# codelion/adaptive-classifier

Measured on NVIDIA B200. Metric: queries/sec predict() bert-base 128-tok, 1M x 768 prototypes, higher is better.
Workload: dtype f16

## Files before the change

### adaptive_classifier_b200/csrc/api.cu

```cuda
#include "common.cuh"
#include <cstdarg>
#include <cudaTypedefs.h>
#include <atomic>
#include <mutex>
#include <vector>

namespace ac {

static thread_local char g_err[512] = "";

void set_error(const char *fmt, ...) {
    va_list ap;
    va_start(ap, fmt);
    vsnprintf(g_err, sizeof(g_err), fmt, ap);
    va_end(ap);
}

int check_cuda(cudaError_t e, const char *what) {
    if (e == cudaSuccess) return AC_OK;
    set_error("CUDA error %d (%s) at %s", static_cast<int>(e), cudaGetErrorString(e), what);
    return AC_E_CUDA;
}

static std::atomic<long long> g_launches{0};
// ... 50 lines not shown
        if (cudaGetDevice(&dev) != cudaSuccess) return 148;
        if (cudaDeviceGetAttribute(&n, cudaDevAttrMultiProcessorCount, dev) != cudaSuccess || n <= 0) n = 148;
    }
    return n;
}

int make_tmap_2d(CUtensorMap *out, const void *gptr, int elem_bytes, uint64_t rows, uint64_t cols,
                 uint64_t row_stride_bytes, uint32_t box_rows, uint32_t box_cols) {
    static PFN_cuTensorMapEncodeTiled_v12000 encode = nullptr;
    static std::once_flag once;
    std::call_once(once, [] {
        void *fn = nullptr;
        cudaDriverEntryPointQueryResult qres;
        if (cudaGetDriverEntryPoint("cuTensorMapEncodeTiled", &fn, cudaEnableDefault, &qres) == cudaSuccess &&
            qres == cudaDriverEntryPointSuccess)
            encode = reinterpret_cast<PFN_cuTensorMapEncodeTiled_v12000>(fn);
    });
    if (!encode) {
        set_error("cuTensorMapEncodeTiled entry point not available (no CUDA driver?)");
        return AC_E_CUDA;
    }
    AC_REQUIRE((reinterpret_cast<uintptr_t>(gptr) & 15) == 0 && row_stride_bytes % 16 == 0,
               "make_tmap_2d: base pointer and row stride must be 16-byte aligned");
    AC_REQUIRE(box_cols * static_cast<uint32_t>(elem_bytes) == 128 && box_rows <= 256,
               "make_tmap_2d: box must be 128 bytes wide and <= 256 rows");
    const CUtensorMapDataType dt = (elem_bytes == 4) ? CU_TENSOR_MAP_DATA_TYPE_FLOAT32 : CU_TENSOR_MAP_DATA_TYPE_FLOAT16;
    cuuint64_t gdim[2] = {cols, rows};
    cuuint64_t gstride[1] = {row_stride_bytes};
    cuuint32_t box[2] = {box_cols, box_rows};
    cuuint32_t estr[2] = {1, 1};
    CUresult r = encode(out, dt, 2, const_cast<void *>(gptr), gdim, gstride, box, estr, CU_TENSOR_MAP_INTERLEAVE_NONE,
                        CU_TENSOR_MAP_SWIZZLE_128B, CU_TENSOR_MAP_L2_PROMOTION_L2_256B,
                        CU_TENSOR_MAP_FLOAT_OOB_FILL_NONE);
    if (r != CUDA_SUCCESS) {
        set_error("cuTensorMapEncodeTiled failed with CUresult %d (rows=%llu cols=%llu)", static_cast<int>(r),
                  static_cast<unsigned long long>(rows), static_cast<unsigned long long>(cols));
        return AC_E_CUDA;
    }
    return AC_OK;
}

int launch_knn_dist_exact(const float *Q, const float *P, int nq, int64_t N, int D, float *Dout, cudaStream_t stream);
int launch_knn_rerank(const float *Q, const float *P, int B, int64_t N, int D, int kc, const int32_t *cand, float *out_d,
                      int64_t *out_i, int64_t row_offset, cudaStream_t stream);
size_t topk_select_workspace(int B, int64_t L, int k);
int topk_select(const float *d, const int64_t *idx, int B, int64_t L, int64_t in_stride, int64_t id_offset, int k,
                float *out_d, int64_t *out_i, void *ws, size_t ws_bytes, cudaStream_t stream, const float *row_gate = nullptr);
size_t knn_tc_workspace(int B, int64_t N, int D, int k);
int knn_tc_search(const float *Q, const float *P, const float *p_sqnorm, const void *p_half, int B, int64_t N, int D, int k,
                  float *out_d, int64_t *out_i, int64_t row_offset, void *ws, size_t ws_bytes, int32_t *stats, cudaStream_t stream);

static int exact_query_block(int B, int64_t N) {
    const int64_t budget = 256ll << 20;
    int64_t qb = budget / (4 * (N > 0 ? N : 1));
    if (qb < 1) qb = 1;
// ... 120 lines not shown
```

### adaptive_classifier_b200/csrc/common.cuh

```cuda
#pragma once

#include <cuda_runtime.h>
#include <cuda.h>
#include <stdint.h>
#include <stdio.h>
#include <string.h>
#include <string>

#include "../../include/adaptive_b200.h"

namespace ac {

void set_error(const char *fmt, ...);
int check_cuda(cudaError_t e, const char *what);

#define AC_CUDA(call)                                                \
    do {                                                             \
        int _rc = ::ac::check_cuda((call), #call);                   \
        if (_rc != 0) return _rc;                                    \
    } while (0)

#define AC_REQUIRE(cond, ...)                                        \
    do {                                                             \
        if (!(cond)) {                                               \
// ... 21 lines not shown

__device__ __forceinline__ uint32_t smem_u32(const void *p) {
    return static_cast<uint32_t>(__cvta_generic_to_shared(p));
}

__device__ __forceinline__ float round_tf32(float x) {
    uint32_t u = __float_as_uint(x);
    u += 0x0FFFu + ((u >> 13) & 1u);
    u &= 0xFFFFE000u;
    return __uint_as_float(u);
}

__device__ __forceinline__ float warp_sum(float v) {
#pragma unroll
    for (int o = 16; o > 0; o >>= 1) v += __shfl_xor_sync(0xffffffffu, v, o);
    return v;
}
__device__ __forceinline__ float warp_max(float v) {
#pragma unroll
    for (int o = 16; o > 0; o >>= 1) v = fmaxf(v, __shfl_xor_sync(0xffffffffu, v, o));
    return v;
}

__device__ __forceinline__ void mbar_init(uint64_t *bar, uint32_t count) {
    asm volatile("mbarrier.init.shared::cta.b64 [%0], %1;" ::"r"(smem_u32(bar)), "r"(count));
}
__device__ __forceinline__ void fence_mbar_init() {
    asm volatile("fence.mbarrier_init.release.cluster;" ::: "memory");
}
__device__ __forceinline__ void mbar_arrive_expect_tx(uint64_t *bar, uint32_t bytes) {
    asm volatile("mbarrier.arrive.expect_tx.shared::cta.b64 _, [%0], %1;" ::"r"(smem_u32(bar)), "r"(bytes)
                 : "memory");
}
__device__ __forceinline__ void mbar_arrive(uint64_t *bar) {
    asm volatile("mbarrier.arrive.shared::cta.b64 _, [%0];" ::"r"(smem_u32(bar)) : "memory");
}
__device__ __forceinline__ bool mbar_try_wait(uint64_t *bar, uint32_t parity) {
    uint32_t ok;
    asm volatile(
        "{\n\t"
        ".reg .pred p;\n\t"
        "mbarrier.try_wait.parity.shared::cta.b64 p, [%1], %2;\n\t"
        "selp.u32 %0, 1, 0, p;\n\t"
        "}"
        : "=r"(ok)
        : "r"(smem_u32(bar)), "r"(parity)
        : "memory");
    return ok != 0;
}
__device__ __forceinline__ void mbar_wait(uint64_t *bar, uint32_t parity) {
    while (!mbar_try_wait(bar, parity)) {
    }
}

__device__ __forceinline__ void tma_prefetch_desc(const CUtensorMap *m) {
    asm volatile("prefetch.tensormap [%0];" ::"l"(reinterpret_cast<uint64_t>(m)) : "memory");
}
__device__ __forceinline__ void tma_load_2d(void *smem_dst, const CUtensorMap *m, uint64_t *bar, int c0, int c1) {
    asm volatile(
        "cp.async.bulk.tensor.2d.shared::cluster.global.tile.mbarrier::complete_tx::bytes [%0], [%1, {%3, %4}], [%2];"
        ::"r"(smem_u32(smem_dst)), "l"(reinterpret_cast<uint64_t>(m)), "r"(smem_u32(bar)), "r"(c0), "r"(c1)
        : "memory");
}
__device__ __forceinline__ void fence_proxy_async_smem() {
    asm volatile("fence.proxy.async.shared::cta;" ::: "memory");
}

__device__ __forceinline__ void tmem_alloc(uint32_t *smem_dst, uint32_t ncols) {
    asm volatile("tcgen05.alloc.cta_group::1.sync.aligned.shared::cta.b32 [%0], %1;" ::"r"(smem_u32(smem_dst)),
                 "r"(ncols)
                 : "memory");
}
__device__ __forceinline__ void tmem_relinquish() {
    asm volatile("tcgen05.relinquish_alloc_permit.cta_group::1.sync.aligned;" ::: "memory");
}
__device__ __forceinline__ void tmem_dealloc(uint32_t taddr, uint32_t ncols) {
    asm volatile("tcgen05.dealloc.cta_group::1.sync.aligned.b32 %0, %1;" ::"r"(taddr), "r"(ncols) : "memory");
}
__device__ __forceinline__ void tc_fence_before() { asm volatile("tcgen05.fence::before_thread_sync;" ::: "memory"); }
__device__ __forceinline__ void tc_fence_after() { asm volatile("tcgen05.fence::after_thread_sync;" ::: "memory"); }

__device__ __forceinline__ void tc_commit(uint64_t *bar) {
    asm volatile("tcgen05.commit.cta_group::1.mbarrier::arrive::one.shared::cluster.b64 [%0];" ::"r"(smem_u32(bar))
                 : "memory");
}

__device__ __forceinline__ uint64_t umma_desc_sw128(uint32_t smem_addr) {
    uint64_t d = 0;
    d |= static_cast<uint64_t>((smem_addr & 0x3FFFFu) >> 4);
// ... 134 lines not shown
```

### adaptive_classifier_b200/csrc/encoder.cu

```cuda
#include "gemm_tc2.cuh"
#include <cuda_fp16.h>
#include <math_constants.h>
#include <vector>

namespace ac {

__device__ __forceinline__ float ex2_approx(float x) {
    float y;
    asm("ex2.approx.ftz.f32 %0, %1;" : "=f"(y) : "f"(x));
    return y;
}
__device__ __forceinline__ float rcp_approx(float x) {
    float y;
    asm("rcp.approx.ftz.f32 %0, %1;" : "=f"(y) : "f"(x));
    return y;
}
__device__ __forceinline__ float gelu_erf(float y) {
    const float ay = fabsf(y);
    const float t = rcp_approx(fmaf(0.3275911f * 0.70710678118654752440f, ay, 1.f));
    float p = fmaf(0.5f * 1.061405429f, t, 0.5f * -1.453152027f);
    p = fmaf(p, t, 0.5f * 1.421413741f);
    p = fmaf(p, t, 0.5f * -0.284496736f);
    p = fmaf(p, t, 0.5f * 0.254829592f);
    const float e = ex2_approx((y * y) * (-0.5f * 1.4426950408889634f));
    const float h = (p * t) * e;
    return fmaxf(y, 0.f) - fabsf(y * h);
}

template <int MODE, bool OUT_HALF, bool VT, bool DEFER = false, int COLS = GEMM_BLOCK_N / 2>
struct EpiLinear {
    static_assert(!DEFER || (OUT_HALF && MODE != 2), "the deferred-LayerNorm consumer epilogues write fp16 operands");
    const float *__restrict__ bias;
    const float *__restrict__ residual;
    void *Y;
    int M, N, ldy;
    int round_out;
    __half *vT;
    int vt_col0, S, S_pad, H;
    const float *__restrict__ c1;
    const float2 *__restrict__ row_stats;

    static constexpr int kUnrollChunks = 4;
    static constexpr int kPrefetchDist = 1;
    struct State {
        float4 res[(MODE == 2) ? 2 : 1][(MODE == 2) ? 8 : 1];
        float mu, r;
    };
    __device__ __forceinline__ float pre(const State &st, float acc, float b, float c1v) const {
        return DEFER ? fmaf(st.r, fmaf(-st.mu, c1v, acc), b) : acc + b;
    }
    __device__ __forceinline__ void begin_cta(State &, int, int) const {}
    __device__ __forceinline__ void end_cta(State &, int, int) const {}

    __device__ __forceinline__ float act(float y) const {
        if (MODE == 1) y = gelu_erf(y);
        return y;
    }

    __device__ __forceinline__ void prefetch(State &st, const GemmTileInfo &ti, int row, int col0, int lane, int buf) const {
        if (DEFER) {
            if (((col0 - ti.n0) & (COLS - 1)) == 0) {
                const float2 ms = (row < M) ? __ldg(row_stats + row) : make_float2(0.f, 0.f);
                st.mu = ms.x;
                st.r = ms.y;
            }
        }
// ... 83 lines not shown
                const float4 b4 = (col + 4 <= N) ? __ldg(reinterpret_cast<const float4 *>(bias + col)) : make_float4(0, 0, 0, 0);
#pragma unroll
                for (int i = 0; i < 4; ++i) {
                    const int rr = r8 + 8 * i;
                    const int grow = row_base + rr;
                    if (grow < M && col + 4 <= N) {
                        const float4 a = *reinterpret_cast<const float4 *>(stage + rr * GEMM_EPI_STAGE_ROW_BYTES + 16 * c);
                        float4 o;
                        o.x = act(a.x + b4.x); o.y = act(a.y + b4.y); o.z = act(a.z + b4.z); o.w = act(a.w + b4.w);
                        if (MODE == 2) {
                            const float4 rs = st.res[buf][half * 4 + i];
                            o.x += rs.x; o.y += rs.y; o.z += rs.z; o.w += rs.w;
                        }
                        if (round_out) { o.x = round_tf32(o.x); o.y = round_tf32(o.y); o.z = round_tf32(o.z); o.w = round_tf32(o.w); }
                        *reinterpret_cast<float4 *>(Yf + static_cast<int64_t>(grow) * ldy + col) = o;
                    }
                }
                __syncwarp();
            }
        }
    }
};

struct EpiResidDefer {
    const float *__restrict__ bias;
    float *y;
    __half *yh;
    const float2 *__restrict__ stats_prev;
    const float *__restrict__ gamma;
    const float *__restrict__ beta;
    float2 *parts;
    int64_t part_stride;
    int M, N, ld;

    static constexpr int kUnrollChunks = 4;
#ifndef AC_RESID_PREFETCH
#define AC_RESID_PREFETCH 1
#endif
    static constexpr int kPrefetchDist = AC_RESID_PREFETCH;
    struct State {
        float4 res[kPrefetchDist + 1][8];
        float2 ms[4];
        float sum[4], sq[4];
    };
    __device__ __forceinline__ void begin_cta(State &, int, int) const {}
    __device__ __forceinline__ void end_cta(State &, int, int) const {}

    __device__ __forceinline__ void prefetch(State &st, const GemmTileInfo &ti, int, int col0, int lane, int buf) const {
        const int row_base = ti.m0 + ((threadIdx.x >> 5) & 3) * 32;
        const int r8 = lane >> 2, c = lane & 3;
        if (((col0 - ti.n0) & (GEMM_BLOCK_N / 2 - 1)) == 0) {
#pragma unroll
            for (int i = 0; i < 4; ++i) {
                const int grow = row_base + r8 + 8 * i;
                st.ms[i] = (grow < M) ? __ldg(stats_prev + grow) : make_float2(0.f, 0.f);
                st.sum[i] = 0.f;
                st.sq[i] = 0.f;
            }
        }
#pragma unroll
        for (int half = 0; half < 2; ++half) {
            const int col = col0 + 16 * half + 4 * c;
// ... 45 lines not shown
                    *reinterpret_cast<uint2 *>(yh + static_cast<int64_t>(grow) * ld + col) = pk;
                    st.sum[i] += (o.x + o.y) + (o.z + o.w);
                    st.sq[i] += (o.x * o.x + o.y * o.y) + (o.z * o.z + o.w * o.w);
                }
            }
            __syncwarp();
        }
        if (((col0 - ti.n0) & (GEMM_BLOCK_N / 2 - 1)) == GEMM_BLOCK_N / 2 - 32) {
            const int part = col0 / (GEMM_BLOCK_N / 2);
#pragma unroll
            for (int i = 0; i < 4; ++i) {
                float s = st.sum[i], q = st.sq[i];
                s += __shfl_xor_sync(0xffffffffu, s, 1);
                q += __shfl_xor_sync(0xffffffffu, q, 1);
                s += __shfl_xor_sync(0xffffffffu, s, 2);
                q += __shfl_xor_sync(0xffffffffu, q, 2);
                const int grow = row_base + r8 + 8 * i;
                if (c == 0 && grow < M) parts[static_cast<int64_t>(part) * part_stride + grow] = make_float2(s, q);
            }
        }
    }
};

__global__ void ln_stats_kernel(const float2 *__restrict__ parts, int nparts, int64_t part_stride, int rows, int H, float eps,
                                float2 *__restrict__ stats) {
    const int row = blockIdx.x * blockDim.x + threadIdx.x;
    if (row >= rows) return;
    float s = 0.f, q = 0.f;
    for (int p = 0; p < nparts; ++p) {
        const float2 v = parts[static_cast<int64_t>(p) * part_stride + row];
        s += v.x;
        q += v.y;
    }
    const float mu = s / static_cast<float>(H);
    const float var = fmaxf(q / static_cast<float>(H) - mu * mu, 0.f);
    stats[row] = make_float2(mu, 1.f / sqrtf(var + eps));
}

__global__ void fill_stats_identity_kernel(float2 *__restrict__ stats, int64_t n) {
    const int64_t i = static_cast<int64_t>(blockIdx.x) * blockDim.x + threadIdx.x;
    if (i < n) stats[i] = make_float2(0.f, 1.f);
}
__global__ void fill_value_kernel(float *__restrict__ p, int n, float v) {
    const int i = blockIdx.x * blockDim.x + threadIdx.x;
    if (i < n) p[i] = v;
}
// ... 501 lines not shown
}

}

using namespace ac;

struct ac_encoder {
    ac_encoder_config cfg;
    float *word = nullptr, *pos = nullptr, *type = nullptr, *emb_ln_w = nullptr, *emb_ln_b = nullptr;
    std::vector<__half *> wqkv_d, wo, w1_d, w2;
    std::vector<float *> c1qkv, c0qkv, c1f, c0f, bo, ln1w, ln1b, b2, ln2w, ln2b;
    __half *w1_last = nullptr;
    float *b1_last = nullptr;
    float *x = nullptr, *tmp = nullptr;
    __half *xh = nullptr, *qk = nullptr, *vT = nullptr, *ctx = nullptr, *ffn = nullptr;
    size_t T = 0;
    size_t vt_elems = 0;
    size_t Bc = 0;
    float *x_cls = nullptr, *tmp_cls = nullptr;
    __half *xh_cls = nullptr, *ctx_cls = nullptr, *ffn_cls = nullptr;
    CUtensorMap m_xh_cls, m_ctx_cls, m_ffn_cls;
    CUtensorMap m_xh, m_ctx, m_ffn, m_qk_att, m_vt_att;
    int vt_B = -1, vt_S = -1;
    std::vector<CUtensorMap> p_wqkv_d, p_wo, p_w1_d, p_w2;
    CUtensorMap p_w1_last;
    float2 *stats_a = nullptr, *stats_b = nullptr, *stats_id = nullptr, *parts = nullptr;
    float *ones = nullptr, *zeros = nullptr;
    std::vector<void *> allocs;
    int last_B = 0, last_S = 0;
    bool last_cls_only = false;
    const float *last_hidden = nullptr;
};

static int launch_cls_normalize(const float *x, int B, int S, int H, float *out, cudaStream_t s) {
    const int wpb = 8;
    cls_normalize_kernel<<<(B + wpb - 1) / wpb, wpb * 32, 0, s>>>(x, B, S, H, out);
    AC_LAUNCH_CHECK();
    return AC_OK;
}

static int launch_attention(ac_encoder *e, const int32_t *mask, int B, int S, cudaStream_t s) {
    const ac_encoder_config &c = e->cfg;
    const int H = c.hidden;
    static bool att_attr[64] = {};
    int dev = 0;
    AC_CUDA(cudaGetDevice(&dev));
// ... 137 lines not shown
    TRY(make_tmap_2d(&e->m_ffn, e->ffn, 2, T, I, static_cast<uint64_t>(I) * 2, GEMM_BLOCK_M, 64));
    TRY(make_tmap_2d(&e->m_qk_att, e->qk, 2, T, 2 * H, static_cast<uint64_t>(2 * H) * 2, 128, 64));
    TRY(make_tmap_2d(&e->m_xh_cls, e->xh_cls, 2, e->Bc, H, static_cast<uint64_t>(H) * 2, GEMM_BLOCK_M, 64));
    TRY(make_tmap_2d(&e->m_ctx_cls, e->ctx_cls, 2, e->Bc, H, static_cast<uint64_t>(H) * 2, GEMM_BLOCK_M, 64));
    TRY(make_tmap_2d(&e->m_ffn_cls, e->ffn_cls, 2, e->Bc, I, static_cast<uint64_t>(I) * 2, GEMM_BLOCK_M, 64));
    e->p_wqkv_d.resize(L); e->p_wo.resize(L); e->p_w1_d.resize(L); e->p_w2.resize(L);
    for (int l = 0; l < L; ++l) {
        TRY(make_tmap_2d(&e->p_wqkv_d[l], e->wqkv_d[l], 2, 3 * H, H, static_cast<uint64_t>(H) * 2, GEMM2_B_ROWS, 64));
        TRY(make_tmap_2d(&e->p_wo[l], e->wo[l], 2, H, H, static_cast<uint64_t>(H) * 2, GEMM2_B_ROWS, 64));
        TRY(make_tmap_2d(&e->p_w1_d[l], e->w1_d[l], 2, I, H, static_cast<uint64_t>(H) * 2, GEMM2_B_ROWS, 64));
        TRY(make_tmap_2d(&e->p_w2[l], e->w2[l], 2, H, I, static_cast<uint64_t>(I) * 2, GEMM2_B_ROWS, 64));
    }
    if (cfg->cls_only) TRY(make_tmap_2d(&e->p_w1_last, e->w1_last, 2, I, H, static_cast<uint64_t>(H) * 2, GEMM2_B_ROWS, 64));
    TRY(check_cuda(cudaDeviceSynchronize(), "encoder_create sync"));
#undef TRY
    *out = e;
    return AC_OK;
}

using EpiGelu = EpiLinear<1, true, false>;
using EpiResid = EpiLinear<2, false, false>;
using EpiQKVDefer = EpiLinear<0, true, true, true>;
using EpiGeluDefer16 = EpiLinear<1, true, false, true, 64>;

template <class Epi, int kEpiWarps = GEMM_EPI_WARPS>
static int launch_linear(const CUtensorMap &ta, const CUtensorMap &tb, int M, int N, int K, const Epi &epi, cudaStream_t s) {
    return launch_gemm_tc2<Epi, false, GEMM_KIND_F16, kEpiWarps>(ta, tb, M, N, K, epi, s);
}

extern "C" int ac_encoder_forward_cls(ac_encoder *e, const int32_t *ids, const int32_t *mask, const int32_t *type_ids,
                                      int B, int S, float *out_unit_cls, ac_stream_t stream) {
    AC_REQUIRE(e && ids && out_unit_cls, "ac_encoder_forward_cls: null argument");
    AC_REQUIRE(B > 0 && S > 0, "ac_encoder_forward_cls: B=%d S=%d", B, S);
    if (S > 512) {
        set_error("ac_encoder_forward_cls: S=%d > 512 is not supported (the reference truncates at max_length = 512)", S);
        return AC_E_UNSUPPORTED;
    }
    AC_REQUIRE(static_cast<int64_t>(B) * S <= e->cfg.max_tokens, "ac_encoder_forward_cls: B*S=%lld exceeds max_tokens=%d",
               static_cast<long long>(B) * S, e->cfg.max_tokens);
    AC_REQUIRE(S <= e->cfg.max_pos, "ac_encoder_forward_cls: S exceeds max_position_embeddings");
    cudaStream_t s = static_cast<cudaStream_t>(stream);
    const ac_encoder_config &c = e->cfg;
    const int H = c.hidden, I = c.intermediate, M = B * S;
    const int S_pad = (S + 7) / 8 * 8;
    AC_REQUIRE(static_cast<size_t>(B) * H * S_pad <= e->vt_elems,
               "ac_encoder_forward_cls: B=%d sequences of S=%d exceed the transposed-V workspace; split the batch", B, S);
    int rc;
    if (e->vt_B != B || e->vt_S != S) {
        if ((rc = make_tmap_2d(&e->m_vt_att, e->vT, 2, static_cast<uint64_t>(B) * H, S_pad, static_cast<uint64_t>(S_pad) * 2, 64, 64)))
            return rc;
        e->vt_B = B; e->vt_S = S;
    }
    const int wpb = 8;
    const int row_blocks = (M + wpb - 1) / wpb;
    const int nparts = H / 128;
    const int64_t pstride = static_cast<int64_t>(e->T);

    embed_ln_kernel<<<row_blocks, wpb * 32, 0, s>>>(ids, type_ids, e->word, e->pos, e->type, e->emb_ln_w, e->emb_ln_b,
                                                    c.ln_eps, B, S, H, c.arch, c.pad_idx, c.vocab, c.max_pos,
                                                    c.type_vocab, e->x, e->xh);
    AC_LAUNCH_CHECK();
    const float *pg = e->ones, *pb = e->zeros;
    const float2 *st_in = e->stats_id;
    for (int l = 0; l < c.layers; ++l) {
        EpiQKVDefer eq{e->c0qkv[l], nullptr, e->qk, M, 3 * H, 2 * H, 0, e->vT, 2 * H, S, S_pad, H, e->c1qkv[l], st_in};
        if ((rc = launch_linear(e->m_xh, e->p_wqkv_d[l], M, 3 * H, H, eq, s))) return rc;
        if ((rc = launch_attention(e, mask, B, S, s))) return rc;
        if (l == c.layers - 1 && c.cls_only && static_cast<size_t>(B) <= e->Bc) {
            const int cb = (B + wpb - 1) / wpb;
            if (l == 0)
                gather_cls_kernel<<<cb, wpb * 32, 0, s>>>(e->ctx, e->x, B, S, H, e->ctx_cls, e->x_cls);
            else
                gather_cls_ln_kernel<<<cb, wpb * 32, 0, s>>>(e->ctx, e->x, B, S, H, pg, pb, c.ln_eps, e->ctx_cls, e->x_cls);
            AC_LAUNCH_CHECK();
            EpiResid eo{e->bo[l], e->x_cls, e->tmp_cls, B, H, H, 0, nullptr, 0, 0, 0, 0};
            if ((rc = launch_linear(e->m_ctx_cls, e->p_wo[l], B, H, H, eo, s))) return rc;
            layernorm_kernel<<<cb, wpb * 32, 0, s>>>(e->tmp_cls, e->ln1w[l], e->ln1b[l], c.ln_eps, B, H, e->x_cls, e->xh_cls);
            AC_LAUNCH_CHECK();
            EpiGelu e1{e->b1_last, nullptr, e->ffn_cls, B, I, I, 0, nullptr, 0, 0, 0, 0};
            if ((rc = launch_linear(e->m_xh_cls, e->p_w1_last, B, I, H, e1, s))) return rc;
            EpiResid e2{e->b2[l], e->x_cls, e->tmp_cls, B, H, H, 0, nullptr, 0, 0, 0, 0};
            if ((rc = launch_linear(e->m_ffn_cls, e->p_w2[l], B, H, I, e2, s))) return rc;
            layernorm_kernel<<<cb, wpb * 32, 0, s>>>(e->tmp_cls, e->ln2w[l], e->ln2b[l], c.ln_eps, B, H, e->x_cls, nullptr);
            AC_LAUNCH_CHECK();
            if ((rc = launch_cls_normalize(e->x_cls, B, 1, H, out_unit_cls, s))) return rc;
            e->last_B = B;
            e->last_S = S;
            e->last_cls_only = true;
            return AC_OK;
        }
        EpiResidDefer eo{e->bo[l], e->x, e->xh, st_in, pg, pb, e->parts, pstride, M, H, H};
        if ((rc = launch_linear(e->m_ctx, e->p_wo[l], M, H, H, eo, s))) return rc;
        ln_stats_kernel<<<(M + 255) / 256, 256, 0, s>>>(e->parts, nparts, pstride, M, H, c.ln_eps, e->stats_b);
        AC_LAUNCH_CHECK();
        EpiGeluDefer16 e1{e->c0f[l], nullptr, e->ffn, M, I, I, 0, nullptr, 0, 0, 0, 0, e->c1f[l], e->stats_b};
        if ((rc = launch_linear<EpiGeluDefer16, 16>(e->m_xh, e->p_w1_d[l], M, I, H, e1, s))) return rc;
        EpiResidDefer e2{e->b2[l], e->x, e->xh, e->stats_b, e->ln1w[l], e->ln1b[l], e->parts, pstride, M, H, H};
        if ((rc = launch_linear(e->m_ffn, e->p_w2[l], M, H, I, e2, s))) return rc;
        ln_stats_kernel<<<(M + 255) / 256, 256, 0, s>>>(e->parts, nparts, pstride, M, H, c.ln_eps, e->stats_a);
        AC_LAUNCH_CHECK();
        pg = e->ln2w[l];
        pb = e->ln2b[l];
        st_in = e->stats_a;
    }
    layernorm_kernel<<<row_blocks, wpb * 32, 0, s>>>(e->x, pg, pb, c.ln_eps, M, H, e->tmp, nullptr);
    AC_LAUNCH_CHECK();
    if ((rc = launch_cls_normalize(e->tmp, B, S, H, out_unit_cls, s))) return rc;
    e->last_B = B;
    e->last_S = S;
    e->last_cls_only = false;
    e->last_hidden = e->tmp;
    return AC_OK;
}

extern "C" int ac_encoder_last_hidden(ac_encoder *e, float *out, int64_t n_floats, ac_stream_t stream) {
    AC_REQUIRE(e && out, "ac_encoder_last_hidden: null argument");
    AC_REQUIRE(!e->last_cls_only, "ac_encoder_last_hidden: the previous forward computed only the CLS rows of the last layer "
                                  "(create the encoder with cls_only = 0 to keep the full hidden state)");
    const int64_t have = static_cast<int64_t>(e->last_B) * e->last_S * e->cfg.hidden;
    AC_REQUIRE(n_floats <= have, "ac_encoder_last_hidden: asked %lld floats, have %lld", (long long)n_floats, (long long)have);
// ... 42 lines not shown
```

### adaptive_classifier_b200/csrc/gemm_tc2.cuh

```cuda
#pragma once
#include "gemm_tc.cuh"

namespace ac {

constexpr int GEMM2_PAIR_M = 2 * GEMM_BLOCK_M;
constexpr int GEMM2_B_ROWS = GEMM_BLOCK_N / 2;
constexpr int GEMM2_A_STAGE_BYTES = GEMM_BLOCK_M * 128;
constexpr int GEMM2_B_STAGE_BYTES = GEMM2_B_ROWS * 128;
constexpr int GEMM2_STAGE_BYTES = GEMM2_A_STAGE_BYTES + GEMM2_B_STAGE_BYTES;
constexpr int GEMM2_STAGES = 6;
__host__ __device__ constexpr int gemm2_smem_bytes(int stages, int epi_warps = GEMM_EPI_WARPS) {
    return stages * GEMM2_STAGE_BYTES + epi_warps * GEMM_EPI_STAGE_BYTES + 1024  + 512 ;
}
__host__ __device__ constexpr int gemm2_stages_for(int epi_warps) { return epi_warps > 8 ? GEMM2_STAGES - 1 : GEMM2_STAGES; }
static_assert(gemm2_smem_bytes(GEMM2_STAGES) <= 227 * 1024, "stage ring does not fit");
static_assert(gemm2_smem_bytes(gemm2_stages_for(16), 16) <= 227 * 1024, "stage ring does not fit with 16 epilogue warps");
static_assert(GEMM2_A_STAGE_BYTES == GEMM_A_STAGE_BYTES, "A stage layout is shared with the 1-CTA kernel");

enum { PAIR_SITE_PRODUCER_EMPTY = 0, PAIR_SITE_MMA_TMEM_EMPTY = 1, PAIR_SITE_MMA_FULL = 2, PAIR_SITE_EPI_TMEM_FULL = 3 };
__device__ __forceinline__ void mbar_wait_guarded_cluster(uint64_t *bar, uint32_t parity, int site, int index) {
    uint32_t spins = 0;
    while (!mbar_try_wait_cluster(bar, parity)) {
        if (++spins > (1u << 24)) {
            printf("ac: mbarrier watchdog fired (pair kernel, block %d rank %u thread %d, site %d, index %d, parity %u)\n", blockIdx.x,
                   cluster_ctarank(), threadIdx.x, site, index, parity);
            __trap();
        }
    }
}

template <class Epi, bool kMFastest = false, int kKind = GEMM_KIND_TF32, int kStages = GEMM2_STAGES, int kEpiWarps = GEMM_EPI_WARPS>
__global__ void __cluster_dims__(2, 1, 1) __launch_bounds__(64 + 32 * kEpiWarps, 1)
gemm_tc2_kernel(const __grid_constant__ CUtensorMap tmap_a, const __grid_constant__ CUtensorMap tmap_b,
                int M, int N, int K, Epi epi) {
    extern __shared__ uint8_t smem_raw[];
    uint8_t *smem = reinterpret_cast<uint8_t *>((reinterpret_cast<uintptr_t>(smem_raw) + 1023) & ~uintptr_t(1023));
    uint8_t *smem_a = smem;
    uint8_t *smem_b = smem + kStages * GEMM2_A_STAGE_BYTES;
    uint8_t *epi_stage = smem + kStages * GEMM2_STAGE_BYTES;
    static_assert(kEpiWarps == 8 || kEpiWarps == 16, "epilogue warps come in multiples of the 4 TMEM lane quarters");
    constexpr int kColsPerWarp = GEMM_BLOCK_N / (kEpiWarps / 4);
    uint64_t *bars = reinterpret_cast<uint64_t *>(epi_stage + kEpiWarps * GEMM_EPI_STAGE_BYTES);
    uint64_t *full_bar = bars;
    uint64_t *empty_bar = bars + kStages;
    uint64_t *tmem_full = bars + 2 * kStages;
    uint64_t *tmem_empty = bars + 2 * kStages + 2;
    uint32_t *tmem_slot = reinterpret_cast<uint32_t *>(bars + 2 * kStages + 4);

    const int warp = threadIdx.x >> 5;
    const int lane = threadIdx.x & 31;
    const uint32_t rank = cluster_ctarank();
    const int cluster = static_cast<int>(blockIdx.x >> 1);
    const int num_clusters = static_cast<int>(gridDim.x >> 1);
    const int tiles_m = (M + GEMM2_PAIR_M - 1) / GEMM2_PAIR_M;
    const int tiles_n = (N + GEMM_BLOCK_N - 1) / GEMM_BLOCK_N;
    const int num_tiles = tiles_m * tiles_n;
    constexpr int BK = gemm_block_k(kKind);
    const int num_kb = (K + BK - 1) / BK;

    if (warp == 0 && lane == 0) {
        tma_prefetch_desc(&tmap_a);
        tma_prefetch_desc(&tmap_b);
        for (int s = 0; s < kStages; ++s) {
            mbar_init(&full_bar[s], 1);
            mbar_init(&empty_bar[s], 1);
        }
        mbar_init(&tmem_full[0], 1);
        mbar_init(&tmem_full[1], 1);
        mbar_init(&tmem_empty[0], 2 * kEpiWarps);
        mbar_init(&tmem_empty[1], 2 * kEpiWarps);
        fence_mbar_init();
    }
    if (warp == 1) {
        tmem_alloc_pair(tmem_slot, GEMM_TMEM_COLS);
        tmem_relinquish_pair();
    }
    tc_fence_before();
    __syncthreads();
    cluster_sync_all();
    tc_fence_after();
    const uint32_t tmem_base = *tmem_slot;

    if (warp == 0) {
        if (lane == 0) {
            int stage = 0;
            uint32_t phase = 0;
            for (int tile = cluster; tile < num_tiles; tile += num_clusters) {
                const int m0 = (kMFastest ? tile % tiles_m : tile / tiles_n) * GEMM2_PAIR_M + static_cast<int>(rank) * GEMM_BLOCK_M;
                const int n0 = (kMFastest ? tile / tiles_m : tile % tiles_n) * GEMM_BLOCK_N + static_cast<int>(rank) * GEMM2_B_ROWS;
                for (int kb = 0; kb < num_kb; ++kb) {
                    mbar_wait_guarded_cluster(&empty_bar[stage], phase ^ 1, PAIR_SITE_PRODUCER_EMPTY, stage);
                    const uint32_t full_leader = mapa_shared(smem_u32(&full_bar[stage]), 0);
                    if (rank == 0) mbar_arrive_expect_tx(&full_bar[stage], 2 * GEMM2_STAGE_BYTES);
// ... 11 lines not shown
            int acc = 0;
            uint32_t acc_phase = 0;
            for (int tile = cluster; tile < num_tiles; tile += num_clusters) {
                mbar_wait_guarded_cluster(&tmem_empty[acc], acc_phase ^ 1, PAIR_SITE_MMA_TMEM_EMPTY, acc);
                tc_fence_after();
                const uint32_t d_tmem = tmem_base + acc * GEMM_BLOCK_N;
                for (int kb = 0; kb < num_kb; ++kb) {
                    mbar_wait_guarded_cluster(&full_bar[stage], phase, PAIR_SITE_MMA_FULL, stage);
                    tc_fence_after();
                    const uint64_t a_desc = umma_desc_sw128(smem_u32(smem_a + stage * GEMM2_A_STAGE_BYTES));
                    const uint64_t b_desc = umma_desc_sw128(smem_u32(smem_b + stage * GEMM2_B_STAGE_BYTES));
#pragma unroll
                    for (int k = 0; k < GEMM_BLOCK_K / GEMM_UMMA_K; ++k) {
                        if (kKind == GEMM_KIND_F16) umma_f16_pair(d_tmem, a_desc + 2 * k, b_desc + 2 * k, idesc, (kb | k) != 0);
                        else umma_tf32_pair(d_tmem, a_desc + 2 * k, b_desc + 2 * k, idesc, (kb | k) != 0);
                    }
                    tc_commit_pair(&empty_bar[stage], 0x3);
                    if (++stage == kStages) { stage = 0; phase ^= 1; }
                }
                tc_commit_pair(&tmem_full[acc], 0x3);
                if (++acc == 2) { acc = 0; acc_phase ^= 1; }
            }
        }
    } else {
        const int q = warp & 3;
        const int cpart = (warp - 2) >> 2;
        typename Epi::State est;
        epi.begin_cta(est, q, lane);
        int acc = 0;
        uint32_t acc_phase = 0;
        int it = 0;
        for (int tile = cluster; tile < num_tiles; tile += num_clusters, ++it) {
            GemmTileInfo ti;
            ti.m0 = (kMFastest ? tile % tiles_m : tile / tiles_n) * GEMM2_PAIR_M + static_cast<int>(rank) * GEMM_BLOCK_M;
            ti.n0 = (kMFastest ? tile / tiles_m : tile % tiles_n) * GEMM_BLOCK_N;
            ti.tile_iter = it;
            const int row = ti.m0 + q * 32 + lane;
            const int c_lo = cpart * kColsPerWarp;
            constexpr int kDist = Epi::kPrefetchDist, kBufs = kDist + 1, kChunks = kColsPerWarp / 32;
#pragma unroll
            for (int d = 0; d < kDist; ++d)
                if (d < kChunks) epi.prefetch(est, ti, row, ti.n0 + c_lo + 32 * d, lane, d % kBufs);
            mbar_wait_guarded_cluster(&tmem_full[acc], acc_phase, PAIR_SITE_EPI_TMEM_FULL, acc);
            tc_fence_after();
            const uint32_t taddr = tmem_base + (static_cast<uint32_t>(q * 32) << 16) + acc * GEMM_BLOCK_N;
#pragma unroll (Epi::kUnrollChunks)
            for (int ci = 0; ci < kChunks; ++ci) {
                const int c = c_lo + 32 * ci;
                if (ci + kDist < kChunks) epi.prefetch(est, ti, row, ti.n0 + c + 32 * kDist, lane, (ci + kDist) % kBufs);
                uint32_t r[32];
                tmem_ld_32x32(taddr + c, r);
                tmem_ld_wait();
                float v[32];
#pragma unroll
                for (int j = 0; j < 32; ++j) v[j] = __uint_as_float(r[j]);
                epi.tile(est, ti, row, ti.n0 + c, v, epi_stage + (warp - 2) * GEMM_EPI_STAGE_BYTES, lane, ci % kBufs, taddr + c);
            }
            tc_fence_before();
            __syncwarp();
            if (lane == 0) mbar_arrive_cluster(mapa_shared(smem_u32(&tmem_empty[acc]), 0));
            if (++acc == 2) { acc = 0; acc_phase ^= 1; }
        }
        epi.end_cta(est, q, lane);
    }

    tc_fence_before();
    __syncthreads();
    cluster_sync_all();
    if (warp == 1) {
        tc_fence_after();
        tmem_dealloc_pair(tmem_base, GEMM_TMEM_COLS);
    }
}

template <class Epi, bool kMFastest = false, int kKind = GEMM_KIND_TF32, int kEpiWarps = GEMM_EPI_WARPS>
int launch_gemm_tc2(const CUtensorMap &ta, const CUtensorMap &tb, int M, int N, int K, const Epi &epi,
                    cudaStream_t stream, int max_ctas = 0, int prof_cls = PROF_GEMM_LINEAR, double prof_bytes = 0.0) {
    constexpr int kStg = gemm2_stages_for(kEpiWarps);
    constexpr int smem = gemm2_smem_bytes(kStg, kEpiWarps);
    auto kern = gemm_tc2_kernel<Epi, kMFastest, kKind, kStg, kEpiWarps>;
    static bool attr_set[64] = {};
    int dev = 0;
    AC_CUDA(cudaGetDevice(&dev));
    if (dev < 0 || dev >= 64 || !attr_set[dev]) {
        AC_CUDA(cudaFuncSetAttribute(kern, cudaFuncAttributeMaxDynamicSharedMemorySize, smem));
        if (dev >= 0 && dev < 64) attr_set[dev] = true;
    }
    const int tiles = ((M + GEMM2_PAIR_M - 1) / GEMM2_PAIR_M) * ((N + GEMM_BLOCK_N - 1) / GEMM_BLOCK_N);
    int clusters = sm_count() / 2;
    if (max_ctas > 0 && max_ctas / 2 < clusters) clusters = max_ctas / 2;
    if (tiles < clusters) clusters = tiles;
    if (clusters <= 0) return AC_OK;
    const int slot = prof_begin(prof_cls, 2.0 * M * static_cast<double>(N) * K, prof_bytes, stream);
    kern<<<2 * clusters, 64 + 32 * kEpiWarps, smem, stream>>>(ta, tb, M, N, K, epi);
    prof_end(slot, stream);
    AC_LAUNCH_CHECK();
    return AC_OK;
}

}
```

Before: 34310.

## Stream residual through TMA loads/stores in attention-output GEMM epilogue

Adds a residual-streaming epilogue path to the paired-CTA tcgen05 GEMM for the attention output projection. The residual tile is loaded by TMA into a per-warp slot ring, combined in shared memory, and the fp32 and fp16 outputs are written back with TMA bulk stores instead of per-thread global loads and stores. The TMEM buffer is released earlier, and the stage count is now derived from the epilogue's shared-memory footprint. In exchange the extra epilogue smem may reduce pipeline stages, and the code adds swizzle-variant tensor maps and more barrier bookkeeping.

```diff
diff --git a/adaptive_classifier_b200/csrc/api.cu b/adaptive_classifier_b200/csrc/api.cu
--- a/adaptive_classifier_b200/csrc/api.cu
+++ b/adaptive_classifier_b200/csrc/api.cu
@@ -96,15 +96,18 @@
     }
     AC_REQUIRE((reinterpret_cast<uintptr_t>(gptr) & 15) == 0 && row_stride_bytes % 16 == 0,
                "make_tmap_2d: base pointer and row stride must be 16-byte aligned");
-    AC_REQUIRE(box_cols * static_cast<uint32_t>(elem_bytes) == 128 && box_rows <= 256,
-               "make_tmap_2d: box must be 128 bytes wide and <= 256 rows");
+    const uint32_t box_bytes = box_cols * static_cast<uint32_t>(elem_bytes);
+    AC_REQUIRE((box_bytes == 32 || box_bytes == 64 || box_bytes == 128) && box_rows <= 256,
+               "make_tmap_2d: box must be 32, 64 or 128 bytes wide and <= 256 rows");
+    const CUtensorMapSwizzle swz = box_bytes == 128 ? CU_TENSOR_MAP_SWIZZLE_128B
+                                   : box_bytes == 64 ? CU_TENSOR_MAP_SWIZZLE_64B : CU_TENSOR_MAP_SWIZZLE_32B;
     const CUtensorMapDataType dt = (elem_bytes == 4) ? CU_TENSOR_MAP_DATA_TYPE_FLOAT32 : CU_TENSOR_MAP_DATA_TYPE_FLOAT16;
     cuuint64_t gdim[2] = {cols, rows};
     cuuint64_t gstride[1] = {row_stride_bytes};
     cuuint32_t box[2] = {box_cols, box_rows};
     cuuint32_t estr[2] = {1, 1};
     CUresult r = encode(out, dt, 2, const_cast<void *>(gptr), gdim, gstride, box, estr, CU_TENSOR_MAP_INTERLEAVE_NONE,
-                        CU_TENSOR_MAP_SWIZZLE_128B, CU_TENSOR_MAP_L2_PROMOTION_L2_256B,
+                        swz, CU_TENSOR_MAP_L2_PROMOTION_L2_256B,
                         CU_TENSOR_MAP_FLOAT_OOB_FILL_NONE);
     if (r != CUDA_SUCCESS) {
         set_error("cuTensorMapEncodeTiled failed with CUresult %d (rows=%llu cols=%llu)", static_cast<int>(r),
diff --git a/adaptive_classifier_b200/csrc/common.cuh b/adaptive_classifier_b200/csrc/common.cuh
--- a/adaptive_classifier_b200/csrc/common.cuh
+++ b/adaptive_classifier_b200/csrc/common.cuh
@@ -67,6 +67,18 @@
     return v;
 }
 
+__device__ __forceinline__ float4 lds128(uint32_t addr) {
+    float4 v;
+    asm volatile("ld.shared.v4.f32 {%0, %1, %2, %3}, [%4];" : "=f"(v.x), "=f"(v.y), "=f"(v.z), "=f"(v.w) : "r"(addr));
+    return v;
+}
+__device__ __forceinline__ void sts128(uint32_t addr, float4 v) {
+    asm volatile("st.shared.v4.f32 [%0], {%1, %2, %3, %4};" ::"r"(addr), "f"(v.x), "f"(v.y), "f"(v.z), "f"(v.w));
+}
+__device__ __forceinline__ void sts128(uint32_t addr, uint4 v) {
+    asm volatile("st.shared.v4.b32 [%0], {%1, %2, %3, %4};" ::"r"(addr), "r"(v.x), "r"(v.y), "r"(v.z), "r"(v.w));
+}
+
 __device__ __forceinline__ void mbar_init(uint64_t *bar, uint32_t count) {
     asm volatile("mbarrier.init.shared::cta.b64 [%0], %1;" ::"r"(smem_u32(bar)), "r"(count));
 }
@@ -110,6 +122,17 @@
 __device__ __forceinline__ void fence_proxy_async_smem() {
     asm volatile("fence.proxy.async.shared::cta;" ::: "memory");
 }
+__device__ __forceinline__ void tma_store_2d(const CUtensorMap *m, const void *smem_src, int c0, int c1) {
+    asm volatile("cp.async.bulk.tensor.2d.global.shared::cta.tile.bulk_group [%0, {%2, %3}], [%1];"
+                 ::"l"(reinterpret_cast<uint64_t>(m)), "r"(smem_u32(smem_src)), "r"(c0), "r"(c1)
+                 : "memory");
+}
+__device__ __forceinline__ void bulk_commit_group() { asm volatile("cp.async.bulk.commit_group;" ::: "memory"); }
+template <int N>
+__device__ __forceinline__ void bulk_wait_group_read() {
+    asm volatile("cp.async.bulk.wait_group.read %0;" ::"n"(N) : "memory");
+}
+__device__ __forceinline__ void bulk_wait_group_all() { asm volatile("cp.async.bulk.wait_group 0;" ::: "memory"); }
 
 __device__ __forceinline__ void tmem_alloc(uint32_t *smem_dst, uint32_t ncols) {
     asm volatile("tcgen05.alloc.cta_group::1.sync.aligned.shared::cta.b32 [%0], %1;" ::"r"(smem_u32(smem_dst)),
diff --git a/adaptive_classifier_b200/csrc/encoder.cu b/adaptive_classifier_b200/csrc/encoder.cu
--- a/adaptive_classifier_b200/csrc/encoder.cu
+++ b/adaptive_classifier_b200/csrc/encoder.cu
@@ -42,6 +42,8 @@
 
     static constexpr int kUnrollChunks = 4;
     static constexpr int kPrefetchDist = 1;
+    static constexpr int kResidSlots = 0;
+    static constexpr int kWarpSmemBytes = GEMM_EPI_STAGE_BYTES;
     struct State {
         float4 res[(MODE == 2) ? 2 : 1][(MODE == 2) ? 8 : 1];
         float mu, r;
@@ -171,7 +173,7 @@
     }
 };
 
-struct EpiResidDefer {
+struct EpiResidDeferReg {
     const float *__restrict__ bias;
     float *y;
     __half *yh;
@@ -183,10 +185,9 @@
     int M, N, ld;
 
     static constexpr int kUnrollChunks = 4;
-#ifndef AC_RESID_PREFETCH
-#define AC_RESID_PREFETCH 1
-#endif
-    static constexpr int kPrefetchDist = AC_RESID_PREFETCH;
+    static constexpr int kPrefetchDist = 1;
+    static constexpr int kResidSlots = 0;
+    static constexpr int kWarpSmemBytes = GEMM_EPI_STAGE_BYTES;
     struct State {
         float4 res[kPrefetchDist + 1][8];
         float2 ms[4];
@@ -278,6 +279,67 @@
     }
 };
 
+template <int kSlots>
+struct EpiResidDefer {
+    const float *__restrict__ bias;
+    const float2 *__restrict__ stats_prev;
+    const float *__restrict__ gamma;
+    const float *__restrict__ beta;
+    float2 *parts;
+    int64_t part_stride;
+    int M, N;
+
+    static constexpr int kResidSlots = kSlots;
+    static constexpr int kWarpSmemBytes = kSlots * GEMM2_RES_CHUNK_BYTES + 2 * GEMM2_RES_HALF_BYTES;
+    struct State {
+        float mu, r;
+        float sum, sq;
+    };
+
+    __device__ __forceinline__ void begin_row(State &st, int row) const {
+        const float2 ms = (row < M) ? __ldg(stats_prev + row) : make_float2(0.f, 0.f);
+        st.mu = ms.x;
+        st.r = ms.y;
+        st.sum = 0.f;
+        st.sq = 0.f;
+    }
+
+    __device__ __forceinline__ void chunk(State &st, int col0, const float (&v)[32], uint8_t *slot, uint8_t *half, int lane) const {
+        if (col0 >= N) return;
+        const uint32_t yrow = smem_u32(slot) + lane * 128;
+        const uint32_t hrow = smem_u32(half) + lane * 64;
+#pragma unroll
+        for (int k = 0; k < 4; ++k) {
+            uint32_t pk[4];
+#pragma unroll
+            for (int jj = 0; jj < 2; ++jj) {
+                const int j = 2 * k + jj;
+                const uint32_t p = yrow + 16 * (j ^ (lane & 7));
+                const float4 rs = lds128(p);
+                const float4 b4 = __ldg(reinterpret_cast<const float4 *>(bias + col0 + 4 * j));
+                const float4 g4 = __ldg(reinterpret_cast<const float4 *>(gamma + col0 + 4 * j));
+                const float4 e4 = __ldg(reinterpret_cast<const float4 *>(beta + col0 + 4 * j));
+                float4 o;
+                o.x = (v[4 * j] + b4.x) + fmaf((rs.x - st.mu) * st.r, g4.x, e4.x);
+                o.y = (v[4 * j + 1] + b4.y) + fmaf((rs.y - st.mu) * st.r, g4.y, e4.y);
+                o.z = (v[4 * j + 2] + b4.z) + fmaf((rs.z - st.mu) * st.r, g4.z, e4.z);
+                o.w = (v[4 * j + 3] + b4.w) + fmaf((rs.w - st.mu) * st.r, g4.w, e4.w);
+                sts128(p, o);
+                st.sum += (o.x + o.y) + (o.z + o.w);
+                st.sq += (o.x * o.x + o.y * o.y) + (o.z * o.z + o.w * o.w);
+                const __half2 h0 = __floats2half2_rn(o.x, o.y), h1 = __floats2half2_rn(o.z, o.w);
+                pk[2 * jj] = *reinterpret_cast<const uint32_t *>(&h0);
+                pk[2 * jj + 1] = *reinterpret_cast<const uint32_t *>(&h1);
+            }
+            sts128(hrow + 16 * (k ^ ((lane >> 1) & 3)), make_uint4(pk[0], pk[1], pk[2], pk[3]));
+        }
+    }
+
+    __device__ __forceinline__ void end_row(const State &st, int row, int col_part0) const {
+        if (row < M && col_part0 < N) parts[static_cast<int64_t>(col_part0 / (GEMM_BLOCK_N / 2)) * part_stride + row] = make_float2(st.sum, st.sq);
+    }
+};
+
 __global__ void ln_stats_kernel(const float2 *__restrict__ parts, int nparts, int64_t part_stride, int rows, int H, float eps,
                                 float2 *__restrict__ stats) {
     const int row = blockIdx.x * blockDim.x + threadIdx.x;
@@ -825,6 +887,8 @@
     CUtensorMap m_xh_cls, m_ctx_cls, m_ffn_cls;
     CUtensorMap m_xh, m_ctx, m_ffn, m_qk_att, m_vt_att;
     int vt_B = -1, vt_S = -1;
+    CUtensorMap m_x_res, m_xh_res;
+    int res_M = -1;
     std::vector<CUtensorMap> p_wqkv_d, p_wo, p_w1_d, p_w2;
     CUtensorMap p_w1_last;
     float2 *stats_a = nullptr, *stats_b = nullptr, *stats_id = nullptr, *parts = nullptr;
@@ -1008,10 +1072,13 @@
 using EpiResid = EpiLinear<2, false, false>;
 using EpiQKVDefer = EpiLinear<0, true, true, true>;
 using EpiGeluDefer16 = EpiLinear<1, true, false, true, 64>;
+using EpiResidOut = EpiResidDefer<3>;
+using EpiResidFfn2 = EpiResidDeferReg;
 
 template <class Epi, int kEpiWarps = GEMM_EPI_WARPS>
-static int launch_linear(const CUtensorMap &ta, const CUtensorMap &tb, int M, int N, int K, const Epi &epi, cudaStream_t s) {
-    return launch_gemm_tc2<Epi, false, GEMM_KIND_F16, kEpiWarps>(ta, tb, M, N, K, epi, s);
+static int launch_linear(const CUtensorMap &ta, const CUtensorMap &tb, int M, int N, int K, const Epi &epi, cudaStream_t s,
+                         const CUtensorMap *tres = nullptr, const CUtensorMap *tres16 = nullptr) {
+    return launch_gemm_tc2<Epi, false, GEMM_KIND_F16, kEpiWarps>(ta, tb, M, N, K, epi, s, 0, PROF_GEMM_LINEAR, 0.0, tres, tres16);
 }
 
 extern "C" int ac_encoder_forward_cls(ac_encoder *e, const int32_t *ids, const int32_t *mask, const int32_t *type_ids,
@@ -1036,6 +1103,11 @@
         if ((rc = make_tmap_2d(&e->m_vt_att, e->vT, 2, static_cast<uint64_t>(B) * H, S_pad, static_cast<uint64_t>(S_pad) * 2, 64, 64)))
             return rc;
         e->vt_B = B; e->vt_S = S;
+    }
+    if (e->res_M != M) {
+        if ((rc = make_tmap_2d(&e->m_x_res, e->x, 4, M, H, static_cast<uint64_t>(H) * 4, 32, 32))) return rc;
+        if ((rc = make_tmap_2d(&e->m_xh_res, e->xh, 2, M, H, static_cast<uint64_t>(H) * 2, 32, 32))) return rc;
+        e->res_M = M;
     }
     const int wpb = 8;
     const int row_blocks = (M + wpb - 1) / wpb;
@@ -1075,13 +1147,13 @@
             e->last_cls_only = true;
             return AC_OK;
         }
-        EpiResidDefer eo{e->bo[l], e->x, e->xh, st_in, pg, pb, e->parts, pstride, M, H, H};
-        if ((rc = launch_linear(e->m_ctx, e->p_wo[l], M, H, H, eo, s))) return rc;
+        EpiResidOut eo{e->bo[l], st_in, pg, pb, e->parts, pstride, M, H};
+        if ((rc = launch_linear(e->m_ctx, e->p_wo[l], M, H, H, eo, s, &e->m_x_res, &e->m_xh_res))) return rc;
         ln_stats_kernel<<<(M + 255) / 256, 256, 0, s>>>(e->parts, nparts, pstride, M, H, c.ln_eps, e->stats_b);
         AC_LAUNCH_CHECK();
         EpiGeluDefer16 e1{e->c0f[l], nullptr, e->ffn, M, I, I, 0, nullptr, 0, 0, 0, 0, e->c1f[l], e->stats_b};
         if ((rc = launch_linear<EpiGeluDefer16, 16>(e->m_xh, e->p_w1_d[l], M, I, H, e1, s))) return rc;
-        EpiResidDefer e2{e->b2[l], e->x, e->xh, e->stats_b, e->ln1w[l], e->ln1b[l], e->parts, pstride, M, H, H};
+        EpiResidFfn2 e2{e->b2[l], e->x, e->xh, e->stats_b, e->ln1w[l], e->ln1b[l], e->parts, pstride, M, H, H};
         if ((rc = launch_linear(e->m_ffn, e->p_w2[l], M, H, I, e2, s))) return rc;
         ln_stats_kernel<<<(M + 255) / 256, 256, 0, s>>>(e->parts, nparts, pstride, M, H, c.ln_eps, e->stats_a);
         AC_LAUNCH_CHECK();
diff --git a/adaptive_classifier_b200/csrc/gemm_tc2.cuh b/adaptive_classifier_b200/csrc/gemm_tc2.cuh
--- a/adaptive_classifier_b200/csrc/gemm_tc2.cuh
+++ b/adaptive_classifier_b200/csrc/gemm_tc2.cuh
@@ -9,15 +9,21 @@
 constexpr int GEMM2_B_STAGE_BYTES = GEMM2_B_ROWS * 128;
 constexpr int GEMM2_STAGE_BYTES = GEMM2_A_STAGE_BYTES + GEMM2_B_STAGE_BYTES;
 constexpr int GEMM2_STAGES = 6;
-__host__ __device__ constexpr int gemm2_smem_bytes(int stages, int epi_warps = GEMM_EPI_WARPS) {
-    return stages * GEMM2_STAGE_BYTES + epi_warps * GEMM_EPI_STAGE_BYTES + 1024  + 512 ;
-}
-__host__ __device__ constexpr int gemm2_stages_for(int epi_warps) { return epi_warps > 8 ? GEMM2_STAGES - 1 : GEMM2_STAGES; }
-static_assert(gemm2_smem_bytes(GEMM2_STAGES) <= 227 * 1024, "stage ring does not fit");
-static_assert(gemm2_smem_bytes(gemm2_stages_for(16), 16) <= 227 * 1024, "stage ring does not fit with 16 epilogue warps");
+constexpr int GEMM2_SMEM_MAX = 227 * 1024;
+__host__ __device__ constexpr int gemm2_smem_bytes(int stages, int epi_warps, int epi_warp_bytes) {
+    return stages * GEMM2_STAGE_BYTES + epi_warps * epi_warp_bytes + 1024  + 512 ;
+}
+__host__ __device__ constexpr int gemm2_stages_for(int epi_warps, int epi_warp_bytes) {
+    const int fit = (GEMM2_SMEM_MAX - gemm2_smem_bytes(0, epi_warps, epi_warp_bytes)) / GEMM2_STAGE_BYTES;
+    return fit < GEMM2_STAGES ? fit : GEMM2_STAGES;
+}
 static_assert(GEMM2_A_STAGE_BYTES == GEMM_A_STAGE_BYTES, "A stage layout is shared with the 1-CTA kernel");
 
-enum { PAIR_SITE_PRODUCER_EMPTY = 0, PAIR_SITE_MMA_TMEM_EMPTY = 1, PAIR_SITE_MMA_FULL = 2, PAIR_SITE_EPI_TMEM_FULL = 3 };
+constexpr int GEMM2_RES_CHUNK_BYTES = 32 * 32 * 4;
+constexpr int GEMM2_RES_HALF_BYTES = 32 * 32 * 2;
+
+enum { PAIR_SITE_PRODUCER_EMPTY = 0, PAIR_SITE_MMA_TMEM_EMPTY = 1, PAIR_SITE_MMA_FULL = 2, PAIR_SITE_EPI_TMEM_FULL = 3,
+       PAIR_SITE_EPI_RESID_FULL = 4 };
 __device__ __forceinline__ void mbar_wait_guarded_cluster(uint64_t *bar, uint32_t parity, int site, int index) {
     uint32_t spins = 0;
     while (!mbar_try_wait_cluster(bar, parity)) {
@@ -32,7 +38,8 @@
 template <class Epi, bool kMFastest = false, int kKind = GEMM_KIND_TF32, int kStages = GEMM2_STAGES, int kEpiWarps = GEMM_EPI_WARPS>
 __global__ void __cluster_dims__(2, 1, 1) __launch_bounds__(64 + 32 * kEpiWarps, 1)
 gemm_tc2_kernel(const __grid_constant__ CUtensorMap tmap_a, const __grid_constant__ CUtensorMap tmap_b,
-                int M, int N, int K, Epi epi) {
+                const __grid_constant__ CUtensorMap tmap_res, const __grid_constant__ CUtensorMap tmap_res16, int M, int N, int K,
+                Epi epi) {
     extern __shared__ uint8_t smem_raw[];
     uint8_t *smem = reinterpret_cast<uint8_t *>((reinterpret_cast<uintptr_t>(smem_raw) + 1023) & ~uintptr_t(1023));
     uint8_t *smem_a = smem;
@@ -40,12 +47,16 @@
     uint8_t *epi_stage = smem + kStages * GEMM2_STAGE_BYTES;
     static_assert(kEpiWarps == 8 || kEpiWarps == 16, "epilogue warps come in multiples of the 4 TMEM lane quarters");
     constexpr int kColsPerWarp = GEMM_BLOCK_N / (kEpiWarps / 4);
-    uint64_t *bars = reinterpret_cast<uint64_t *>(epi_stage + kEpiWarps * GEMM_EPI_STAGE_BYTES);
+    constexpr int kResSlots = Epi::kResidSlots;
+    static_assert(Epi::kWarpSmemBytes % 1024 == 0 || kResSlots == 0, "residual slots keep the 1024-byte swizzle alignment");
+    static_assert((2 * kStages + 5 + kEpiWarps * kResSlots) * 8 <= 512, "barriers do not fit");
+    uint64_t *bars = reinterpret_cast<uint64_t *>(epi_stage + kEpiWarps * Epi::kWarpSmemBytes);
     uint64_t *full_bar = bars;
     uint64_t *empty_bar = bars + kStages;
     uint64_t *tmem_full = bars + 2 * kStages;
     uint64_t *tmem_empty = bars + 2 * kStages + 2;
     uint32_t *tmem_slot = reinterpret_cast<uint32_t *>(bars + 2 * kStages + 4);
+    uint64_t *res_full = bars + 2 * kStages + 5;
 
     const int warp = threadIdx.x >> 5;
     const int lane = threadIdx.x & 31;
@@ -69,6 +80,7 @@
         mbar_init(&tmem_full[1], 1);
         mbar_init(&tmem_empty[0], 2 * kEpiWarps);
         mbar_init(&tmem_empty[1], 2 * kEpiWarps);
+        for (int i = 0; i < kEpiWarps * kResSlots; ++i) mbar_init(&res_full[i], 1);
         fence_mbar_init();
     }
     if (warp == 1) {
@@ -126,6 +138,75 @@
                 if (++acc == 2) { acc = 0; acc_phase ^= 1; }
             }
         }
+    } else if constexpr (kResSlots > 0) {
+        static_assert(kEpiWarps == 8, "one warp drains one 128-column part of the row statistics");
+        static_assert(Epi::kWarpSmemBytes == kResSlots * GEMM2_RES_CHUNK_BYTES + 2 * GEMM2_RES_HALF_BYTES, "warp smem layout");
+        constexpr int kChunks = kColsPerWarp / 32;
+        const int q = warp & 3;
+        const int c_lo = ((warp - 2) >> 2) * kColsPerWarp;
+        uint8_t *wsm = epi_stage + (warp - 2) * Epi::kWarpSmemBytes;
+        uint8_t *half_stage = wsm + kResSlots * GEMM2_RES_CHUNK_BYTES;
+        uint64_t *rfull = res_full + (warp - 2) * kResSlots;
+        const int nchunks = (num_tiles - cluster + num_clusters - 1) / num_clusters * kChunks;
+        auto chunk_row0 = [&](int g) {
+            const int tile = cluster + (g / kChunks) * num_clusters;
+            return (kMFastest ? tile % tiles_m : tile / tiles_n) * GEMM2_PAIR_M + static_cast<int>(rank) * GEMM_BLOCK_M + q * 32;
+        };
+        auto chunk_col0 = [&](int g) {
+            const int tile = cluster + (g / kChunks) * num_clusters;
+            return (kMFastest ? tile / tiles_m : tile % tiles_n) * GEMM_BLOCK_N + c_lo + 32 * (g % kChunks);
+        };
+        auto load = [&](int g) {
+            if (g >= nchunks) return;
+            const int s = g % kResSlots;
+            mbar_arrive_expect_tx(&rfull[s], GEMM2_RES_CHUNK_BYTES);
+            tma_load_2d(wsm + s * GEMM2_RES_CHUNK_BYTES, &tmap_res, &rfull[s], chunk_col0(g), chunk_row0(g));
+        };
+        if (lane == 0) {
+            tma_prefetch_desc(&tmap_res);
+            tma_prefetch_desc(&tmap_res16);
+            for (int g = 0; g < kResSlots - 1; ++g) load(g);
+        }
+        typename Epi::State est;
+        int acc = 0;
+        uint32_t acc_phase = 0;
+        for (int g = 0; g < nchunks; ++g) {
+            const int ci = g % kChunks, row0 = chunk_row0(g), col0 = chunk_col0(g);
+            if (ci == 0) {
+                epi.begin_row(est, row0 + lane);
+                mbar_wait_guarded_cluster(&tmem_full[acc], acc_phase, PAIR_SITE_EPI_TMEM_FULL, acc);
+                tc_fence_after();
+            }
+            uint32_t r[32];
+            tmem_ld_32x32(tmem_base + (static_cast<uint32_t>(q * 32) << 16) + acc * GEMM_BLOCK_N + c_lo + 32 * ci, r);
+            tmem_ld_wait();
+            if (ci == kChunks - 1) {
+                tc_fence_before();
+                __syncwarp();
+                if (lane == 0) mbar_arrive_cluster(mapa_shared(smem_u32(&tmem_empty[acc]), 0));
+                if (++acc == 2) { acc = 0; acc_phase ^= 1; }
+            }
+            float v[32];
+#pragma unroll
+            for (int j = 0; j < 32; ++j) v[j] = __uint_as_float(r[j]);
+            const int s = g % kResSlots;
+            uint8_t *slot = wsm + s * GEMM2_RES_CHUNK_BYTES;
+            uint8_t *hst = half_stage + (g & 1) * GEMM2_RES_HALF_BYTES;
+            mbar_wait_guarded_cluster(&rfull[s], (g / kResSlots) & 1, PAIR_SITE_EPI_RESID_FULL, s);
+            epi.chunk(est, col0, v, slot, hst, lane);
+            if (ci == kChunks - 1) epi.end_row(est, row0 + lane, col0 - 32 * ci);
+            fence_proxy_async_smem();
+            __syncwarp();
+            if (lane == 0) {
+                tma_store_2d(&tmap_res, slot, col0, row0);
+                tma_store_2d(&tmap_res16, hst, col0, row0);
+                bulk_commit_group();
+                bulk_wait_group_read<1>();
+                load(g - 1 + kResSlots);
+            }
+            __syncwarp();
+        }
+        if (lane == 0) bulk_wait_group_all();
     } else {
         const int q = warp & 3;
         const int cpart = (warp - 2) >> 2;
@@ -158,7 +239,7 @@
                 float v[32];
 #pragma unroll
                 for (int j = 0; j < 32; ++j) v[j] = __uint_as_float(r[j]);
-                epi.tile(est, ti, row, ti.n0 + c, v, epi_stage + (warp - 2) * GEMM_EPI_STAGE_BYTES, lane, ci % kBufs, taddr + c);
+                epi.tile(est, ti, row, ti.n0 + c, v, epi_stage + (warp - 2) * Epi::kWarpSmemBytes, lane, ci % kBufs, taddr + c);
             }
             tc_fence_before();
             __syncwarp();
@@ -179,9 +260,12 @@
 
 template <class Epi, bool kMFastest = false, int kKind = GEMM_KIND_TF32, int kEpiWarps = GEMM_EPI_WARPS>
 int launch_gemm_tc2(const CUtensorMap &ta, const CUtensorMap &tb, int M, int N, int K, const Epi &epi,
-                    cudaStream_t stream, int max_ctas = 0, int prof_cls = PROF_GEMM_LINEAR, double prof_bytes = 0.0) {
-    constexpr int kStg = gemm2_stages_for(kEpiWarps);
-    constexpr int smem = gemm2_smem_bytes(kStg, kEpiWarps);
+                    cudaStream_t stream, int max_ctas = 0, int prof_cls = PROF_GEMM_LINEAR, double prof_bytes = 0.0,
+                    const CUtensorMap *tres = nullptr, const CUtensorMap *tres16 = nullptr) {
+    AC_REQUIRE(Epi::kResidSlots == 0 || (tres && tres16), "launch_gemm_tc2: the residual-streaming epilogue needs its two maps");
+    constexpr int kStg = gemm2_stages_for(kEpiWarps, Epi::kWarpSmemBytes);
+    constexpr int smem = gemm2_smem_bytes(kStg, kEpiWarps, Epi::kWarpSmemBytes);
+    static_assert(kStg >= 2 && smem <= GEMM2_SMEM_MAX, "stage ring does not fit next to the epilogue's shared memory");
     auto kern = gemm_tc2_kernel<Epi, kMFastest, kKind, kStg, kEpiWarps>;
     static bool attr_set[64] = {};
     int dev = 0;
@@ -196,7 +280,7 @@
     if (tiles < clusters) clusters = tiles;
     if (clusters <= 0) return AC_OK;
     const int slot = prof_begin(prof_cls, 2.0 * M * static_cast<double>(N) * K, prof_bytes, stream);
-    kern<<<2 * clusters, 64 + 32 * kEpiWarps, smem, stream>>>(ta, tb, M, N, K, epi);
+    kern<<<2 * clusters, 64 + 32 * kEpiWarps, smem, stream>>>(ta, tb, tres ? *tres : ta, tres16 ? *tres16 : ta, M, N, K, epi);
     prof_end(slot, stream);
     AC_LAUNCH_CHECK();
     return AC_OK;
```

Result: faster. 35290 (median of 6 runs) (+2.9%).
